# I2PC/xmipp3

Measured on AMD Instinct MI355X. Metric: particles/s projection-matched+reconstructed, 256x256 box, higher is better.
Workload: dtype f32 (coarse search, gridding) + f64 (exact re-score, shifts, finaliser)

## Files before the change

### xmipp3_amd/csrc/xh_pm.hip

```cpp
#include "xh_common.h"
#include "xh_fft.h"
#include "xh_fftreg.h"
#include "xh_plan.h"
#include "xh_bspline.h"
#include <algorithm>
#include <cmath>
#include <cstring>
#include <type_traits>

namespace {
const double kPI = 3.14159265358979323846;
const double kTWOPI = 6.2831853071795864769;

struct Layout {
    int D, Ri, Ro, nrings, nsamples, ncoef, N, nk;
    std::vector<int> nsam, soff, coff;
};

void make_layout(Layout &L, int D, int Ri, int Ro)
{
    L.D = D; L.Ri = Ri; L.Ro = Ro; L.nrings = Ro - Ri + 1;
    L.nsam.resize(L.nrings); L.soff.resize(L.nrings); L.coff.resize(L.nrings);
    L.nsamples = L.ncoef = 0;
    for (int r = 0; r < L.nrings; ++r) {
// ... 34 lines not shown
    int p0, np;
    int qoff, nq;
    int row0;
    int rowstride;
};
}

struct xh_pm {
    xh_ctx *ctx;
    Layout L;
    int nrefs, logM, M;
    double tau_rel, scale;
    size_t chunk_rows;
    XhBuf d_sin, d_cos, d_ringOfSample, d_nsam, d_soff, d_coff, d_rstart, d_ringW;
    XhBuf d_tw32, d_tw64;
    XhBuf d_refs64, d_refsB, d_refSigma, d_refCoef, d_refCoef32;
    XhBuf d_W32;
    XhBuf d_Wfull, d_vperm;
    int R1, R2, R3;
    XhBuf d_chirp, d_vhat;
    XhBuf d_csN;
    XhBuf d_WD64;
    XhBuf d_refScale;
    XhPlanBufs<double> planD;
    XhBuf d_coef32, d_polar32, d_A32, d_stat32;
    XhBuf d_trAngles;
    XhBuf d_trScale;
    XhBuf d_cellStart, d_cellSamples, d_cellOrg, d_cellData;
    int ncells;
    XhBuf d_coef64, d_polar64, d_A64, d_stat64;
    XhBuf d_raw, d_rowres, d_desc, d_nbr, d_poff;
    XhBuf d_ambList, d_ambSlot, d_candRow, d_candRes, d_counters, d_offs5d, d_thrLists;
    int ref_threads = 1;
    XhBuf d_t1, d_t2, d_t3;
    int64_t stat_rows, stat_resc_p, stat_resc_r;
    int coefFirst, coefCount;
    hipEvent_t ev[6] = {};
    double stage_ms[8];
    int store_cut;
    int s6_capture;
    int s6_captured;
    int s6_capturedN;
    int s6_fp32;
    double s6_eps;
    long long s6_flagged;
    XhBuf d_firTmp64;
    int tr_chunk_mb;
    int use_prune;
    int use_mask_lists;
    XhBuf d_bpart, d_rowBound, d_rowTail, d_topRows, d_thr, d_survList, d_survSpan, d_highStore;
    int group_high;
    int high_cap;
    int s6_layout;
    int low_pass;
    int64_t stat_pruned;
    int64_t stat_low_in, stat_low_out, stat_low_rows;
    int lastPruneRows;
    int lastLowPass;
    int adaptive_finish;
    int finish_dense;
    int stat_dense_chunks;
    int K0, K0auto, quadsLow;
    XhBuf d_bT, d_aT, d_kboundsLow, d_bTband;
    XhBuf d_firTmp, d_polarPart, d_trPart, d_listMask, d_s6Flag, d_s6List, d_s6Parts, d_s6Meta, d_s6Out;
    XhBuf d_qoff, d_Bpack, d_Apack, d_kbounds;
    int totalQuads;
    ~xh_pm()
    {
        (void)hipSetDevice(ctx->device);
        (void)hipStreamSynchronize(ctx->stream);
        for (hipEvent_t e : ev)
            if (e) (void)hipEventDestroy(e);
    }
};

__device__ __forceinline__ double d_block_sum(double v, double *red)
{
    for (int o = 32; o > 0; o >>= 1) v += __shfl_down(v, o, 64);
    const int lane = threadIdx.x & 63, wv = threadIdx.x >> 6;
    __syncthreads();
    if (lane == 0) red[wv] = v;
    __syncthreads();
    double t = 0;
    const int nw = (blockDim.x + 63) >> 6;
    for (int i = 0; i < nw; ++i) t += red[i];
    return t;
}

template <typename T>
__global__ void __launch_bounds__(256)
k_pm_polar(const T *__restrict__ coefs, T *__restrict__ polar, double *__restrict__ stat,
           const float *__restrict__ sinr, const float *__restrict__ cosr, const short *__restrict__ ringOf,
           const double *__restrict__ ringW, int D, int Ri, int nsamples, double xoff, double yoff,
           const int *__restrict__ count, int nt, const double *__restrict__ offs, int nparts, double *__restrict__ partial)
{
    __shared__ double red[8];
    const int slot = blockIdx.x / nparts, part = blockIdx.x - slot * nparts;
    if (count && slot / nt >= *count) return;
    const T *c = coefs + (size_t)(slot / nt) * D * D;
    if (offs) { xoff = offs[2 * (slot % nt)]; yoff = offs[2 * (slot % nt) + 1]; }
    const T minp = (T)(-(D / 2)), maxp = (T)(-(D / 2) + D - 1);
    const T eps = (T)1e-6;
    double sw = 0, swv = 0, swv2 = 0;
    const int per = (nsamples + nparts - 1) / nparts;
    const int iEnd = min(nsamples, (part + 1) * per);
    for (int i = part * per + threadIdx.x; i < iEnd; i += blockDim.x) {
        T xp = (T)sinr[i] + (T)xoff;
        T yp = (T)cosr[i] + (T)yoff;
        if (xp < minp - eps || xp > maxp + eps) xp = d_realwrap<T>(xp, minp - (T)0.5, maxp + (T)0.5);
        if (yp < minp - eps || yp > maxp + eps) yp = d_realwrap<T>(yp, minp - (T)0.5, maxp + (T)0.5);
        const T v = d_interp<T>(c, D, xp, yp);
        polar[(size_t)slot * nsamples + i] = v;
        const double w = ringW[ringOf[i]];
        const double dv = (double)v;
        sw += w; swv += w * dv; swv2 += w * dv * dv;
// ... 494 lines not shown
        for (int p = 0; p < PT; ++p)
#pragma unroll
            for (int q = 0; q < QT; ++q) {
                acc[p][q][0] = fmaf(a[p].x, b[q].x, acc[p][q][0]);
                acc[p][q][1] = fmaf(a[p].x, b[q].y, acc[p][q][1]);
                acc[p][q][2] = fmaf(a[p].y, b[q].x, acc[p][q][2]);
                acc[p][q][3] = fmaf(a[p].y, b[q].y, acc[p][q][3]);
            }
    }
#pragma unroll
    for (int p = 0; p < PT; ++p)
#pragma unroll
        for (int q = 0; q < QT; ++q)
            if (p < d.np && q < d.nq) {
                const size_t row = (size_t)d.row0 + (size_t)p * d.rowstride + q;
                raw[row * nk + k] = make_float4(acc[p][q][0], acc[p][q][1], acc[p][q][2], acc[p][q][3]);
            }
}


typedef float xh_f32x16 __attribute__((ext_vector_type(16)));

__global__ void k_pm_pack_tiles(const xh_cf *__restrict__ src, float4 *__restrict__ dst, const int *__restrict__ qoff,
                                const int *__restrict__ rstart, const int *__restrict__ coff, const int *__restrict__ nsam,
                                int nrings, int ncoef, int nk, int totalQuads, int nitems, const int *__restrict__ ids,
                                int quadLimit)
{
    const size_t gid = (size_t)blockIdx.x * blockDim.x + threadIdx.x;
    const int l = gid & 63;
    const size_t rest = gid >> 6;
    const int quad = rest % totalQuads;
    const int tile = rest / totalQuads;
    if ((size_t)tile * 16 >= (size_t)((nitems + 15) / 16) * 16) return;
    if (quad >= quadLimit) return;
    int lo = 0, hi = nk - 1;
    while (lo < hi) { const int mid = (lo + hi + 1) >> 1; if (qoff[mid] <= quad) lo = mid; else hi = mid - 1; }
    const int k = lo, q = quad - qoff[k];
    const int item = tile * 16 + ((l & 31) >> 1), part = l & 1;
    float v[4];
#pragma unroll
    for (int t = 0; t < 4; ++t) {
        const int ring = rstart[k] + 8 * q + 2 * t + (l >> 5);
        float x = 0.f;
        if (item < nitems && ring < nrings && k <= nsam[ring] / 2) {
            const int it = ids ? ids[item] : item;
            const xh_cf c = src[(size_t)it * ncoef + coff[ring] + k];
            x = part ? c.y : c.x;
        }
        v[t] = x;
    }
    dst[gid] = make_float4(v[0], v[1], v[2], v[3]);
}

#define XH_PW2 1
#define XH_KSPLIT 8
#define XH_CT_NQ 4
template <int PT, int QT, bool LDS = false>
__global__ void __launch_bounds__(64 * PT * QT)
k_pm_contract_mfma(const float4 *__restrict__ Apack, const float4 *__restrict__ Bpack, float4 *__restrict__ raw,
                   const int *__restrict__ qoff, const int *__restrict__ kbounds, int nk, int totalQuads, int nparticles,
                   int nq, int nqtiles, int nptiles, float2 *__restrict__ bpart, int rawStride, int kStore)
{
    static_assert(!LDS || (PT == 1 && XH_PW2 == 1 && XH_CT_NQ % QT == 0), "the LDS form shares one particle tile per workgroup");
    const int lane = threadIdx.x & 63, wv = threadIdx.x >> 6;
    int qtile = blockIdx.x * QT + wv % QT;
    const int ptile0 = (blockIdx.y * PT + wv / QT) * XH_PW2;
    const int kBeg = kbounds[blockIdx.z], kEnd = kbounds[blockIdx.z + 1];
    if (!LDS && qtile >= nqtiles) return;
    const int qtileStore = qtile;
    qtile = min(qtile, nqtiles - 1);
    const float4 *A[XH_PW2];
#pragma unroll
    for (int t = 0; t < XH_PW2; ++t) A[t] = Apack + (size_t)min(ptile0 + t, nptiles - 1) * totalQuads * 64 + lane;
    const float4 *B = Bpack + (size_t)qtile * totalQuads * 64 + lane;
    constexpr int STAGE_F4 = LDS ? (XH_CT_NQ + QT * XH_CT_NQ) * 64 : 1;
    __shared__ float4 sOp[2 * STAGE_F4];
    const unsigned sBase = LDS ? (unsigned)(uintptr_t)(const __attribute__((address_space(3))) float4 *)sOp : 0u;
    const int hi = lane >> 5, j = lane & 31;
    const int qj = j >> 1, odd = j & 1;
    const int q = qtileStore * 16 + qj;
    const int lastQuad = qoff[nk] - 1;
    float bndS[XH_PW2][4][2], bndM[XH_PW2][4][2];
#pragma unroll
    for (int t = 0; t < XH_PW2; ++t)
#pragma unroll
        for (int g = 0; g < 4; ++g) { bndS[t][g][0] = bndS[t][g][1] = 0.f; bndM[t][g][0] = bndM[t][g][1] = 0.f; }
    auto modulus = [&](const float4 &o, int k, float &bs, float &bm) {
        const float fsr = o.x - o.w, fsi = o.y + o.z, fmr = o.x + o.w, fmi = o.y - o.z;
        if (k == 0 || k == nk - 1) { bs += fabsf(fsr); bm += fabsf(fmr); }
        else { bs += 2.f * sqrtf(fsr * fsr + fsi * fsi); bm += 2.f * sqrtf(fmr * fmr + fmi * fmi); }
    };
    float4 a0[XH_PW2], a1[XH_PW2], b0, b1;
    const int qFirst = min(qoff[kBeg], lastQuad);
    int curStage = -1;
    const int wvq = __builtin_amdgcn_readfirstlane(wv % QT), qtileU = __builtin_amdgcn_readfirstlane(qtile);
    const int ptileU = __builtin_amdgcn_readfirstlane(min(ptile0, nptiles - 1));
    auto issueStage = [&](int st) {
        const unsigned buf = sBase + (unsigned)(st & 1) * (unsigned)(STAGE_F4 * 16);
        const unsigned off = (unsigned)lane * 16u;
#pragma unroll
        for (int jq = 0; jq < XH_CT_NQ; ++jq) {
            const int qd = min(qFirst + st * XH_CT_NQ + jq, lastQuad);
            const char *gb = reinterpret_cast<const char *>(Bpack) + ((size_t)qtileU * totalQuads + qd) * 1024;
            asm volatile("s_mov_b32 m0, %2\n\ts_nop 0\n\tglobal_load_lds_dwordx4 %0, %1" :: "v"(off), "s"(gb),
                         "s"(buf + (unsigned)(XH_CT_NQ + wvq * XH_CT_NQ + jq) * 1024u) : "memory");
            if (jq % QT == wvq) {
                const char *ga = reinterpret_cast<const char *>(Apack) + ((size_t)ptileU * totalQuads + qd) * 1024;
                asm volatile("s_mov_b32 m0, %2\n\ts_nop 0\n\tglobal_load_lds_dwordx4 %0, %1" :: "v"(off), "s"(ga), "s"(buf + (unsigned)jq * 1024u) : "memory");
            }
        }
    };
    auto fetch = [&](int qd, float4 (&av)[XH_PW2], float4 &bv) {
        if constexpr (!LDS) {
            bv = B[(size_t)qd * 64];
#pragma unroll
            for (int t = 0; t < XH_PW2; ++t) av[t] = A[t][(size_t)qd * 64];
        } else {
            const int rel = qd - qFirst, st = rel / XH_CT_NQ, jq = rel - st * XH_CT_NQ;
            if (st > curStage) {
                asm volatile("s_waitcnt vmcnt(0)" ::: "memory");
                __syncthreads();
                curStage = st;
                issueStage(st + 1);
            }
            const float4 *bufp = sOp + (size_t)(st & 1) * STAGE_F4;
            av[0] = bufp[jq * 64 + lane];
            bv = bufp[(XH_CT_NQ + wvq * XH_CT_NQ + jq) * 64 + lane];
        }
    };
    if constexpr (LDS) issueStage(0);
    fetch(qFirst, a0, b0);
    b1 = b0;
#pragma unroll
    for (int t = 0; t < XH_PW2; ++t) a1[t] = a0[t];
    for (int k0 = kBeg; k0 < kEnd; k0 += 4) {
        xh_f32x16 acc[XH_PW2][4];
#pragma unroll
        for (int kk = 0; kk < 4; ++kk) {
#pragma unroll
            for (int t = 0; t < XH_PW2; ++t)
#pragma unroll
                for (int e = 0; e < 16; ++e) acc[t][kk][e] = 0.f;
            const int k = k0 + kk;
            if (k < kEnd) {
                const int qb = qoff[k], qe = qoff[k + 1];
#define XH_CT_STEP(AC, BC, AN, BN, QN)                                                                        \
                {                                                                                              \
                    const int qn_ = (QN) <= lastQuad ? (QN) : lastQuad;                                        \
                    fetch(qn_, AN, BN);                                                                        \
                    __builtin_amdgcn_sched_barrier(0);                                                         \
                    _Pragma("unroll") for (int t = 0; t < XH_PW2; ++t) {                                       \
                        acc[t][kk] = __builtin_amdgcn_mfma_f32_32x32x2f32(AC[t].x, BC.x, acc[t][kk], 0, 0, 0); \
                        acc[t][kk] = __builtin_amdgcn_mfma_f32_32x32x2f32(AC[t].y, BC.y, acc[t][kk], 0, 0, 0); \
                        acc[t][kk] = __builtin_amdgcn_mfma_f32_32x32x2f32(AC[t].z, BC.z, acc[t][kk], 0, 0, 0); \
                        acc[t][kk] = __builtin_amdgcn_mfma_f32_32x32x2f32(AC[t].w, BC.w, acc[t][kk], 0, 0, 0); \
                    }                                                                                          \
                    __builtin_amdgcn_sched_barrier(0);                                                         \
                }
                for (int qd = qb; qd < qe; qd += 2) {
                    XH_CT_STEP(a0, b0, a1, b1, qd + 1)
                    if (qd + 1 < qe) XH_CT_STEP(a1, b1, a0, b0, qd + 2)
                }
#undef XH_CT_STEP
                if ((qe - qb) & 1) {
                    b0 = b1;
#pragma unroll
                    for (int t = 0; t < XH_PW2; ++t) a0[t] = a1[t];
                }
            }
        }
#pragma unroll
        for (int t = 0; t < XH_PW2; ++t)
#pragma unroll
        for (int g = 0; g < 4; ++g)
#pragma unroll
            for (int h2 = 0; h2 < 2; ++h2) {
                const int r0 = 4 * g + 2 * h2;
                const int pi = 4 * g + 2 * hi + h2;
                const int p = (ptile0 + t) * 16 + pi;
                float mine[4][2], theirs[2][2];
#pragma unroll
                for (int kk = 0; kk < 4; ++kk) { mine[kk][0] = acc[t][kk][r0]; mine[kk][1] = acc[t][kk][r0 + 1]; }
#pragma unroll
                for (int c = 0; c < 2; ++c) {
                    const float s0 = odd ? mine[0][c] : mine[2][c];
                    const float s1 = odd ? mine[1][c] : mine[3][c];
                    theirs[0][c] = __shfl_xor(s0, 1, 64);
                    theirs[1][c] = __shfl_xor(s1, 1, 64);
                }
                if (ptile0 + t < nptiles && p < nparticles && q < nq) {
                    float4 *dst = raw + ((size_t)p * nq + q) * rawStride;
                    const int kA = k0 + (odd ? 2 : 0);
                    float4 o0, o1;
                    if (!odd) {
                        o0 = make_float4(mine[0][0], theirs[0][0], mine[0][1], theirs[0][1]);
                        o1 = make_float4(mine[1][0], theirs[1][0], mine[1][1], theirs[1][1]);
                    } else {
                        o0 = make_float4(theirs[0][0], mine[2][0], theirs[0][1], mine[2][1]);
                        o1 = make_float4(theirs[1][0], mine[3][0], theirs[1][1], mine[3][1]);
                    }
                    if (kA < kEnd && kA < kStore) dst[kA] = o0;
                    if (kA + 1 < kEnd && kA + 1 < kStore) dst[kA + 1] = o1;
                    if (bpart) {
                        if (kA < kEnd) modulus(o0, kA, bndS[t][g][h2], bndM[t][g][h2]);
                        if (kA + 1 < kEnd) modulus(o1, kA + 1, bndS[t][g][h2], bndM[t][g][h2]);
                    }
                }
            }
    }
    if (bpart) {
        const size_t nrowsTotal = (size_t)nparticles * nq;
#pragma unroll
        for (int t = 0; t < XH_PW2; ++t)
#pragma unroll
            for (int g = 0; g < 4; ++g)
#pragma unroll
                for (int h2 = 0; h2 < 2; ++h2) {
                    const float bs = bndS[t][g][h2] + __shfl_xor(bndS[t][g][h2], 1, 64);
                    const float bm = bndM[t][g][h2] + __shfl_xor(bndM[t][g][h2], 1, 64);
                    const int p = (ptile0 + t) * 16 + 4 * g + 2 * hi + h2;
                    if (!odd && ptile0 + t < nptiles && p < nparticles && q < nq)
                        bpart[(size_t)blockIdx.z * nrowsTotal + (size_t)p * nq + q] = make_float2(bs, bm);
                }
    }
}

struct RowRes { float best; int idx; float second; int pad; };

__device__ __forceinline__ void d_top2_insert(float v, int i, float &b, int &bi, float &s)
{
    if (v > b || (v == b && i < bi)) { s = b; b = v; bi = i; }
    else if (v > s) s = v;
}

template <int LOGM>
__global__ void __launch_bounds__(256)
k_pm_idft_max(const float4 *__restrict__ raw, RowRes *__restrict__ res, const xh_cf *__restrict__ W,
              const xh_cf *__restrict__ chirp, const xh_cf *__restrict__ vhat, int N, int nk, int nrows, int lpb)
{
    extern __shared__ __align__(16) unsigned char smem[];
    xh_cf *s = reinterpret_cast<xh_cf *>(smem);
    constexpr int M = 1 << LOGM;
    const int tid = threadIdx.x, nth = blockDim.x;
    const int row0 = blockIdx.x * lpb;
    const int nl = min(lpb, nrows - row0);
    for (int i = tid; i < lpb * M; i += nth) s[i] = xh_cf{0.f, 0.f};
    __syncthreads();
    const int half = N / 2;
    for (int i = tid; i < nl * nk; i += nth) {
        const int l = i / nk, k = i - l * nk;
        const float4 q = raw[(size_t)(row0 + l) * nk + k];
        const float fsr = q.x - q.w, fsi = q.y + q.z;
        const float fmr = q.x + q.w, fmi = q.y - q.z;
        xh_cf *u = s + l * M;
        if (k == 0 || k == half) {
            u[k] = xh_cmul(xh_cf{fsr, fmr}, chirp[k]);
        } else {
            u[k] = xh_cmul(xh_cf{fsr - fmi, fsi + fmr}, chirp[k]);
            u[N - k] = xh_cmul(xh_cf{fsr + fmi, fmr - fsi}, chirp[N - k]);
        }
    }
    __syncthreads();
    xh_fft_dif<float, false>(s, LOGM, lpb, W, LOGM, tid, nth);
    for (int i = tid; i < lpb * M; i += nth) s[i] = xh_cmul(s[i], vhat[i & (M - 1)]);
    __syncthreads();
    xh_fft_dit<float, true>(s, LOGM, lpb, W, LOGM, tid, nth);
    __shared__ float rb[4 * 64], rs[4 * 64];
    __shared__ int ri[4 * 64];
    const int lane = tid & 63, wv = tid >> 6, nw = nth >> 6;
    for (int l = 0; l < nl; ++l) {
        float b = -3.0e38f, sec = -3.0e38f;
        int bi = 0x7fffffff;
        for (int i = tid; i < N; i += nth) {
            const xh_cf z = xh_cmul(s[l * M + i], chirp[i]);
            d_top2_insert(z.x, i, b, bi, sec);
            d_top2_insert(z.y, N + i, b, bi, sec);
// ... 2385 lines not shown
        XH_LAUNCH_CHECK();
        return XH_OK;
    }
    const size_t smem2 = sizeof(T) * ((L.N + 3) & ~3) + sizeof(xh_c2<T>) * L.N;
    hipLaunchKernelGGL((k_pm_ringdft<T>), dim3(L.nrings, (unsigned)nps), dim3(256), smem2, ctx->stream, (const T *)polarBuf.p,
                       (const double *)statBuf.p, (xh_c2<T> *)outBuf.p, (const xh_c2<T> *)twBuf.p,
                       (const int *)pm->d_nsam.p, (const int *)pm->d_soff.p, (const int *)pm->d_coff.p, L.nsamples,
                       L.ncoef, conjugate ? 1 : 0, d_count, nt);
    XH_LAUNCH_CHECK();
    return XH_OK;
}

template <typename T> static int upload(xh_ctx *ctx, XhBuf &b, const std::vector<T> &v)
{
    return xh_buf_upload(ctx, b, v.data(), sizeof(T) * v.size());
}

template <int LOGM>
static void launch_idft(xh_pm *pm, int nrows, int lpb, size_t smem)
{
    hipLaunchKernelGGL((k_pm_idft_max<LOGM>), dim3((nrows + lpb - 1) / lpb), dim3(256), smem, pm->ctx->stream,
                       (const float4 *)pm->d_raw.p, (RowRes *)pm->d_rowres.p, (const xh_cf *)pm->d_W32.p,
                       (const xh_cf *)pm->d_chirp.p, (const xh_cf *)pm->d_vhat.p, pm->L.N, pm->L.nk, nrows, lpb);
}
template <int LOGM>
static void launch_idft_dump(xh_pm *pm, float *d_out, size_t smem)
{
    hipLaunchKernelGGL((k_pm_idft_dump<LOGM>), dim3(1), dim3(256), smem, pm->ctx->stream, (const float4 *)pm->d_raw.p, d_out,
                       (const xh_cf *)pm->d_W32.p, (const xh_cf *)pm->d_chirp.p, (const xh_cf *)pm->d_vhat.p, pm->L.N,
                       pm->L.nk);
}

extern "C" {

static int set_k0(xh_pm *pm, int K0)
{
    const Layout &L = pm->L;
    K0 = std::max(4, std::min(L.nk, (K0 + 3) / 4 * 4));
    std::vector<int> qoff(L.nk + 1);
    XH_HIP(hipMemcpy(qoff.data(), pm->d_qoff.p, sizeof(int) * (L.nk + 1), hipMemcpyDeviceToHost));
    const int quads = qoff[K0];
    std::vector<int> kb(XH_KSPLIT + 1, K0);
    kb[0] = 0;
    for (int sidx = 1; sidx < XH_KSPLIT; ++sidx) {
        const int target = (int)((long long)quads * sidx / XH_KSPLIT);
        int k = 0;
        while (k < K0 && qoff[k] < target) ++k;
        kb[sidx] = std::min(K0, (k + 3) / 4 * 4);
    }
    XH_TRY(xh_buf_reserve(pm->ctx, pm->d_kboundsLow, sizeof(int) * kb.size()));
    XH_HIP(hipMemcpy(pm->d_kboundsLow.p, kb.data(), sizeof(int) * kb.size(), hipMemcpyHostToDevice));
    pm->K0 = K0;
    pm->quadsLow = quads;
    return XH_OK;
}

int xh_pm_create(xh_ctx *ctx, int32_t D, int32_t Ri, int32_t Ro, int32_t nrefs, const float *d_refs,
                 const double *h_Mctf, int32_t paddim, xh_pm **out)
{
    XH_CHECK(ctx && d_refs && out && nrefs > 0, XH_ERR_ARG, "xh_pm_create: bad argument");
    XH_CHECK(h_Mctf == nullptr || (paddim >= D && paddim <= 2048), XH_ERR_UNSUPPORTED,
             "xh_pm_create: the CTF filter size (paddim=%d) must lie in [image size %d, 2048]", paddim, D);
    if (Ri < 1) Ri = 1;
    if (Ro < 0) Ro = (D / 2) - 1;
    XH_CHECK(D >= 8 && Ro >= Ri && Ro < D, XH_ERR_ARG, "xh_pm_create: bad geometry D=%d Ri=%d Ro=%d", D, Ri, Ro);
    XH_HIP(hipSetDevice(ctx->device));
    std::unique_ptr<xh_pm> pm(new xh_pm);
    pm->ctx = ctx;
    pm->nrefs = nrefs;
    make_layout(pm->L, D, Ri, Ro);
    Layout &L = pm->L;
    XH_CHECK(L.nk <= 1024 && L.nrings <= 512, XH_ERR_UNSUPPORTED, "xh_pm_create: Ro=%d gives %d angular frequencies / %d rings; limits are 1024 / 512",
             Ro, L.nk, L.nrings);
    pm->M = 1;
    while (pm->M < 2 * L.N - 1) pm->M <<= 1;
    pm->logM = xh_ilog2(pm->M);
    XH_CHECK(pm->logM >= 6 && pm->logM <= 12, XH_ERR_UNSUPPORTED, "xh_pm_create: convolution length %d outside the supported 64..4096", pm->M);
    pm->scale = 0;
    for (int r = 0; r < L.nrings; ++r) pm->scale += 2. * kPI * (r + Ri);
    pm->tau_rel = D >= 128 ? 2e-6 : 3e-6;
    pm->s6_capture = 0;
    pm->s6_captured = 0;
    pm->s6_capturedN = 0;
    pm->s6_fp32 = 1;
    pm->s6_eps = 6.4e-6;
    pm->s6_flagged = 0;
    pm->use_prune = 1;
    pm->use_mask_lists = 1;
    pm->tr_chunk_mb = 0;
    pm->stat_pruned = 0;
    pm->lastPruneRows = 0;
    pm->adaptive_finish = 1;
    pm->group_high = 1;
    pm->low_pass = 1;
    pm->s6_layout = 1;
    pm->stat_low_in = pm->stat_low_out = pm->stat_low_rows = 0;
    pm->lastLowPass = 0;
    pm->high_cap = 0;
    pm->finish_dense = 0;
    pm->stat_dense_chunks = 0;
    pm->store_cut = 0;
    pm->chunk_rows = 0;
    pm->stat_rows = pm->stat_resc_p = pm->stat_resc_r = 0;
    pm->coefFirst = pm->coefCount = 0;
    for (int i = 0; i < 8; ++i) pm->stage_ms[i] = 0;
    for (int i = 0; i < 6; ++i) (void)hipEventCreate(&pm->ev[i]);
    {
        std::vector<float> sn(L.nsamples), cs(L.nsamples);
        std::vector<short> ringOf(L.nsamples), ringOfCoef(L.ncoef);
        std::vector<xh_cf> tw32(L.nsamples);
        std::vector<xh_cd> tw64(L.nsamples);
        for (int r = 0; r < L.nrings; ++r) {
            const float radius = r + Ri;
            const int n = L.nsam[r];
            const float dphi = kTWOPI / (float)n;
            for (int i = 0; i < n; ++i) {
                const float phi = i * dphi;
                sn[L.soff[r] + i] = std::sin(phi) * radius;
                cs[L.soff[r] + i] = std::cos(phi) * radius;
                ringOf[L.soff[r] + i] = (short)r;
                const long double a = -2.0L * 3.14159265358979323846264338327950288L * i / n;
                tw64[L.soff[r] + i] = xh_cd{(double)cosl(a), (double)sinl(a)};
                tw32[L.soff[r] + i] = xh_cf{(float)cosl(a), (float)sinl(a)};
            }
            for (int k = 0; k <= n / 2; ++k) ringOfCoef[L.coff[r] + k] = (short)r;
        }
        std::vector<int> rstart(L.nk);
        for (int k = 0; k < L.nk; ++k) {
            int r = 0;
            while (r < L.nrings && L.nsam[r] / 2 < k) ++r;
            rstart[k] = r;
        }
        const int M = pm->M, N = L.N;
        std::vector<xh_cf> W32(M / 2), chirp(N), vbr(M);
        for (int j = 0; j < M / 2; ++j) {
            const long double a = -2.0L * 3.14159265358979323846264338327950288L * j / M;
            W32[j] = xh_cf{(float)cosl(a), (float)sinl(a)};
        }
        std::vector<xh_cd> b(M, xh_cd{0., 0.});
        for (int n2 = 0; n2 < N; ++n2) {
            const long long q = ((long long)n2 * n2) % (2LL * N);
            const long double a = 3.14159265358979323846264338327950288L * (long double)q / (long double)N;
            chirp[n2] = xh_cf{(float)cosl(a), (float)sinl(a)};
            const xh_cd v{(double)cosl(a), (double)-sinl(a)};
            b[n2] = v;
            if (n2 > 0) b[M - n2] = v;
        }
        h_fft(b, false);
// ... 137 lines not shown
                                            pm->d_A64, pm->d_stat64, pm->d_tw64, true, 0., 0.));
                if (hipMemcpyAsync((xh_cd *)pm->d_refs64.p + (size_t)r0 * L.ncoef, pm->d_A64.p, sizeof(xh_cd) * (size_t)m * L.ncoef,
                                   hipMemcpyDeviceToDevice, ctx->stream) != hipSuccess ||
                    hipMemcpyAsync((double *)pm->d_refCoef.p + (size_t)r0 * D * D, pm->d_coef64.p, sizeof(double) * (size_t)m * D * D,
                                   hipMemcpyDeviceToDevice, ctx->stream) != hipSuccess ||
                    hipMemcpyAsync(stat.data(), pm->d_stat64.p, sizeof(double) * 2 * m, hipMemcpyDeviceToHost, ctx->stream) != hipSuccess ||
                    hipStreamSynchronize(ctx->stream) != hipSuccess) {
                    xh_set_error("xh_pm_create: reference library copy failed: %s", hipGetErrorString(hipGetLastError()));
                    return XH_ERR_HIP;
                }
                for (int i = 0; i < m; ++i) sig[r0 + i] = stat[2 * i + 1];
            }
            (void)hipStreamSynchronize(ctx->stream);
        }
        XH_CHECK(hipMemcpy(pm->d_refSigma.p, sig.data(), sizeof(double) * nrefs, hipMemcpyHostToDevice) == hipSuccess, XH_ERR_HIP,
                 "xh_pm_create: sigma upload failed");
        XH_TRY(xh_buf_alloc(ctx, pm->d_refScale, sizeof(int2) * nrefs));
        hipLaunchKernelGGL(k_pm_s6_norm_refs, dim3(nrefs), dim3(256), 0, ctx->stream, (const double *)pm->d_refCoef.p, D * D, (int2 *)pm->d_refScale.p);
        XH_CHECK(hipGetLastError() == hipSuccess, XH_ERR_HIP, "xh_pm_create: reference norms failed");
        {
            const size_t total = (size_t)nrefs * L.ncoef;
            hipLaunchKernelGGL(k_pm_pack_refs, dim3((unsigned)((total + 255) / 256)), dim3(256), 0, ctx->stream,
                               (const xh_cd *)pm->d_refs64.p, (xh_cf *)pm->d_refsB.p, (const short *)d_ringOfCoef.p, Ri, L.ncoef, total);
            XH_CHECK(hipGetLastError() == hipSuccess && hipStreamSynchronize(ctx->stream) == hipSuccess, XH_ERR_HIP, "xh_pm_create: pack kernel failed");
        }
        {
            std::vector<int> qoff(L.nk + 1);
            qoff[0] = 0;
            for (int k = 0; k < L.nk; ++k) qoff[k + 1] = qoff[k] + (L.nrings - rstart[k] + 7) / 8;
            pm->totalQuads = qoff[L.nk];
            XH_TRY(upload(ctx, pm->d_qoff, qoff));
            {
                std::vector<int> kb(XH_KSPLIT + 1, L.nk);
                kb[0] = 0;
                for (int sidx = 1; sidx < XH_KSPLIT; ++sidx) {
                    const int target = (int)((long long)pm->totalQuads * sidx / XH_KSPLIT);
                    int k = 0;
                    while (k < L.nk && qoff[k] < target) ++k;
                    kb[sidx] = std::min(L.nk, (k + 3) / 4 * 4);
                }
                XH_TRY(upload(ctx, pm->d_kbounds, kb));
            }
            const int ntiles = (nrefs + 15) / 16;
            const size_t nvec = (size_t)ntiles * pm->totalQuads * 64;
            XH_TRY(xh_buf_alloc(ctx, pm->d_Bpack, nvec * sizeof(float4)));
            {
                hipLaunchKernelGGL(k_pm_pack_tiles, dim3((unsigned)((nvec + 255) / 256)), dim3(256), 0, ctx->stream, (const xh_cf *)pm->d_refsB.p,
                                   (float4 *)pm->d_Bpack.p, (const int *)pm->d_qoff.p, (const int *)pm->d_rstart.p, (const int *)pm->d_coff.p,
                                   (const int *)pm->d_nsam.p, L.nrings, L.ncoef, L.nk, pm->totalQuads, nrefs, (const int *)nullptr, pm->totalQuads);
                XH_CHECK(hipGetLastError() == hipSuccess && hipStreamSynchronize(ctx->stream) == hipSuccess, XH_ERR_HIP, "xh_pm_create: operand packing failed");
            }
            pm->K0 = pm->K0auto = L.nk;
            pm->quadsLow = pm->totalQuads;
            XH_TRY(xh_buf_alloc(ctx, pm->d_bT, sizeof(float) * (size_t)L.nk * nrefs));
            {
                hipLaunchKernelGGL(k_pm_tail_norms, dim3((L.nk + 63) / 64, nrefs), dim3(64), 0, ctx->stream, (const xh_cf *)pm->d_refsB.p,
                                   (float *)pm->d_bT.p, (const int *)pm->d_coff.p, (const int *)pm->d_rstart.p, L.nrings, L.ncoef, L.nk, 0,
                                   nrefs, (size_t)1, (size_t)nrefs);
                std::vector<float> bT((size_t)L.nk * nrefs);
                XH_CHECK(hipGetLastError() == hipSuccess && hipMemcpy(bT.data(), pm->d_bT.p, pm->d_bT.bytes, hipMemcpyDeviceToHost) == hipSuccess, XH_ERR_HIP,
                         "xh_pm_create: reference norms failed");
                {
                    std::vector<double> mean(L.nk, 0.);
                    double all = 0;
                    for (int k = 0; k < L.nk; ++k) {
                        for (int r = 0; r < nrefs; ++r) mean[k] += bT[(size_t)k * nrefs + r];
                        all += mean[k];
                    }
                    double tailSum = 0;
                    int K0 = L.nk;
                    for (int k = L.nk - 1; k >= 0; --k) {
                        tailSum += mean[k];
                        if (!(tailSum <= 1e-5 * all)) break;
                        K0 = k;
                    }
                    K0 = std::min(L.nk, (K0 + 3) / 4 * 4);
                    if (K0 < 8) K0 = 8;
                    if (K0 > (int)(0.6 * L.nk)) K0 = L.nk;
                    pm->K0auto = K0;
                    XH_TRY(set_k0(pm.get(), K0));
                    const int nb = (L.nk + XH_TAIL_BAND - 1) / XH_TAIL_BAND;
                    std::vector<float> bb((size_t)nb * nrefs, 0.f);
                    for (int k = 0; k < L.nk; ++k)
                        for (int r = 0; r < nrefs; ++r) bb[(size_t)(k / XH_TAIL_BAND) * nrefs + r] += bT[(size_t)k * nrefs + r];
                    for (float &v : bb) v *= 1.000002f;
                    XH_TRY(upload(ctx, pm->d_bTband, bb));
                }
            }
        }
    }
    *out = pm.release();
    return XH_OK;
}

int xh_pm_destroy(xh_pm *pm)
{
    delete pm;
    return XH_OK;
}

int xh_pm_info(const xh_pm *pm, int32_t *N, int32_t *ncoef, int32_t *nsamples)
{
    XH_CHECK(pm, XH_ERR_ARG, "null handle");
    if (N) *N = pm->L.N;
    if (ncoef) *ncoef = pm->L.ncoef;
    if (nsamples) *nsamples = pm->L.nsamples;
    return XH_OK;
}

int xh_pm_set_option(xh_pm *pm, const char *name, double value)
{
    XH_CHECK(pm && name, XH_ERR_ARG, "null argument");
    if (!strcmp(name, "tau_rel")) pm->tau_rel = value;
    else if (!strcmp(name, "chunk_rows")) pm->chunk_rows = (size_t)value;
    else if (!strcmp(name, "s6_capture")) pm->s6_capture = (int)value;
    else if (!strcmp(name, "s6_fp32")) pm->s6_fp32 = (int)value;
    else if (!strcmp(name, "s6_eps")) pm->s6_eps = value;
    else if (!strcmp(name, "prune")) pm->use_prune = (int)value;
    else if (!strcmp(name, "mask_lists")) pm->use_mask_lists = (int)value;
    else if (!strcmp(name, "group_high")) pm->group_high = (int)value;
    else if (!strcmp(name, "low_pass")) pm->low_pass = (int)value;
    else if (!strcmp(name, "s6_layout")) pm->s6_layout = (int)value != 0;
    else if (!strcmp(name, "high_cap")) pm->high_cap = (int)value;
    else if (!strcmp(name, "adaptive_finish")) { pm->adaptive_finish = (int)value; pm->finish_dense = value >= 2; }
    else if (!strcmp(name, "threads")) {
        XH_CHECK(value >= 1 && value <= XH_MAX_ORIENT, XH_ERR_ARG, "xh_pm_set_option: threads in [1, %d]", XH_MAX_ORIENT);
        pm->ref_threads = (int)value;
    }
    else if (!strcmp(name, "tr_chunk_mb")) pm->tr_chunk_mb = (int)value;
    else if (!strcmp(name, "k0")) {
        XH_HIP(hipSetDevice(pm->ctx->device));
        XH_HIP(hipStreamSynchronize(pm->ctx->stream));
        XH_TRY(set_k0(pm, value <= 0 ? pm->K0auto : (int)value));
    }
    else { xh_set_error("xh_pm_set_option: unknown option %s", name); return XH_ERR_ARG; }
    return XH_OK;
}

int xh_pm_stage_ms(xh_pm *pm, double *h_ms, int32_t reset)
{
    XH_CHECK(pm && h_ms, XH_ERR_ARG, "null argument");
    for (int i = 0; i < 8; ++i) { h_ms[i] = pm->stage_ms[i]; if (reset) pm->stage_ms[i] = 0; }
    return XH_OK;
}

int xh_pm_two_level_cut(const xh_pm *pm, int32_t *K0, int32_t *nk)
{
    XH_CHECK(pm, XH_ERR_ARG, "null handle");
    if (K0) *K0 = pm->K0;
    if (nk) *nk = pm->L.nk;
    return XH_OK;
}

int xh_pm_rows_pruned(const xh_pm *pm, int64_t *rows_pruned)
{
    XH_CHECK(pm && rows_pruned, XH_ERR_ARG, "null argument");
    *rows_pruned = pm->stat_pruned;
    return XH_OK;
}

int xh_pm_last_coefficients(const xh_pm *pm, const float **d_coefs, int32_t *first, int32_t *count)
{
    XH_CHECK(pm && d_coefs && first && count, XH_ERR_ARG, "null argument");
    *d_coefs = pm->coefCount > 0 ? (const float *)pm->d_coef32.p : nullptr;
    *first = pm->coefFirst;
    *count = pm->coefCount;
    return XH_OK;
}

int xh_pm_last_stats(const xh_pm *pm, int64_t *rows, int64_t *rp, int64_t *rr)
{
    XH_CHECK(pm, XH_ERR_ARG, "null handle");
    if (rows) *rows = pm->stat_rows;
    if (rp) *rp = pm->stat_resc_p;
    if (rr) *rr = pm->stat_resc_r;
    return XH_OK;
}

static int run_rows(xh_pm *pm, int m, const std::vector<int> &poff, const int *d_ids, bool dense, int nq, hipEvent_t evMid = nullptr,
                    const RowMap *prune = nullptr, int nparticles = 0, float tau2 = 0.f, int *d_pruned = nullptr,
                    const unsigned *d_mask = nullptr, int maskW = 0, int listedRows = 0)
{
    xh_ctx *ctx = pm->ctx;
    const Layout &L = pm->L;
    const int nrows = poff[m];
    if (nrows == 0) return XH_OK;
    XH_TRY(xh_buf_reserve(ctx, pm->d_rowres, sizeof(RowRes) * (size_t)nrows));
    XH_CHECK(!dense || nq == pm->nrefs, XH_ERR_STATE, "xh_pm_match: internal error, a dense search covers the whole bank");
    std::vector<BlockDesc> desc;
    if (!dense) {
        for (int p = 0; p < m; ++p)
            for (int q0 = poff[p]; q0 < poff[p + 1]; q0 += 8) {
                BlockDesc d;
                d.p0 = p; d.np = 1; d.qoff = q0; d.nq = std::min(8, poff[p + 1] - q0);
                d.row0 = q0; d.rowstride = 0;
                desc.push_back(d);
            }
        XH_TRY(xh_buf_reserve(ctx, pm->d_desc, sizeof(BlockDesc) * desc.size()));
        XH_HIP(hipMemcpyAsync(pm->d_desc.p, desc.data(), sizeof(BlockDesc) * desc.size(), hipMemcpyHostToDevice, ctx->stream));
        XH_HIP(hipStreamSynchronize(ctx->stream));
    }
    const int nt = ((L.nk + 63) / 64) * 64;
    const bool pruning = dense && prune && pm->use_prune && pm->R1 && nparticles > 0 && nrows % nparticles == 0;
    XH_CHECK(!d_mask || pruning, XH_ERR_STATE, "xh_pm_match: internal error, a masked search must take the pruning path");
    if (pruning) XH_TRY(xh_buf_reserve(ctx, pm->d_bpart, sizeof(float2) * (size_t)XH_KSPLIT * nrows));
    const int K0 = pruning ? pm->K0 : L.nk;
    const bool boundsOnly = pruning && K0 >= L.nk && pm->store_cut >= 0 && pm->store_cut < L.nk;
    const int rawStride = boundsOnly ? pm->store_cut : std::min(K0, L.nk);
    XH_TRY(xh_buf_reserve(ctx, pm->d_raw, sizeof(float4) * std::max<size_t>(1, (size_t)nrows * rawStride)));
    XhHigh H;
    H.A = (const xh_cf *)pm->d_A32.p; H.B = (const xh_cf *)pm->d_refsB.p; H.coff = (const int *)pm->d_coff.p;
    H.rstart = (const int *)pm->d_rstart.p; H.nrings = L.nrings; H.ncoef = L.ncoef; H.K0 = boundsOnly ? rawStride : K0; H.nq = nq; H.zeroHigh = 0; H.rawStride = rawStride;
    H.nk = L.nk;
    H.highStore = nullptr; H.highCap = 0;
    if (dense) {
        const int ptiles = (m + 15) / 16, qtiles = (nq + 15) / 16;
        const size_t nvec = (size_t)ptiles * pm->totalQuads * 64;
        XH_TRY(xh_buf_reserve(ctx, pm->d_Apack, nvec * sizeof(float4)));
        hipLaunchKernelGGL(k_pm_pack_tiles, dim3((unsigned)((nvec + 255) / 256)), dim3(256), 0, ctx->stream, (const xh_cf *)pm->d_A32.p,
                           (float4 *)pm->d_Apack.p, (const int *)pm->d_qoff.p, (const int *)pm->d_rstart.p, (const int *)pm->d_coff.p,
                           (const int *)pm->d_nsam.p, L.nrings, L.ncoef, L.nk, pm->totalQuads, m, (const int *)nullptr,
                           K0 < L.nk ? pm->quadsLow : pm->totalQuads);
        XH_LAUNCH_CHECK();
        const int *kb = (const int *)(K0 < L.nk ? pm->d_kboundsLow.p : pm->d_kbounds.p);
        float2 *bpart = pruning ? (float2 *)pm->d_bpart.p : (float2 *)nullptr;
        if (K0 < L.nk)
            hipLaunchKernelGGL((k_pm_contract_mfma<1, 4, true>), dim3((qtiles + 3) / 4, ptiles, XH_KSPLIT), dim3(256), 0, ctx->stream,
                               (const float4 *)pm->d_Apack.p, (const float4 *)pm->d_Bpack.p, (float4 *)pm->d_raw.p, (const int *)pm->d_qoff.p,
                               kb, L.nk, pm->totalQuads, m, nq, qtiles, ptiles, bpart, rawStride, rawStride);
        else
            hipLaunchKernelGGL((k_pm_contract_mfma<1, 4>), dim3((qtiles + 3) / 4, (ptiles + XH_PW2 - 1) / XH_PW2, XH_KSPLIT), dim3(256), 0, ctx->stream,
                               (const float4 *)pm->d_Apack.p, (const float4 *)pm->d_Bpack.p, (float4 *)pm->d_raw.p, (const int *)pm->d_qoff.p,
                               kb, L.nk, pm->totalQuads, m, nq, qtiles, ptiles, bpart, rawStride, rawStride);
    } else
        hipLaunchKernelGGL((k_pm_contract<1, 8>), dim3((unsigned)desc.size()), dim3(nt), 0, ctx->stream,
                           (const BlockDesc *)pm->d_desc.p, (const xh_cf *)pm->d_A32.p, (const xh_cf *)pm->d_refsB.p, d_ids,
                           (float4 *)pm->d_raw.p, (const int *)pm->d_coff.p, (const int *)pm->d_rstart.p, L.nrings, L.ncoef, L.nk);
    XH_LAUNCH_CHECK();
    if (evMid) XH_HIP(hipEventRecord(evMid, ctx->stream));
    const int lpb = std::max(1, std::min(4, (60 * 1024) / (int)(pm->M * sizeof(xh_cf))));
    const size_t smem = (size_t)lpb * pm->M * sizeof(xh_cf);
    if (pm->R1) {
#define XH_IDFT3(A_, B_, C_)                                                                                  \
    hipLaunchKernelGGL((k_pm_idft_max3<A_, B_, C_>), dim3(grid), dim3(256), 0, ctx->stream, (const float4 *)pm->d_raw.p, \
                       (RowRes *)pm->d_rowres.p, (const xh_cf *)pm->d_Wfull.p, (const xh_cf *)pm->d_chirp.p,       \
                       (const xh_cf *)pm->d_vperm.p, L.N, L.nk, nr, rowList, H, nrDev)
#define XH_IDFT3_ANY()                                  \
    do {                                                \
        if (pm->logM == 9) XH_IDFT3(8, 8, 8);           \
        else if (pm->logM == 10) XH_IDFT3(16, 8, 8);    \
        else XH_IDFT3(16, 16, 8);                       \
    } while (0)
        int nr = nrows;
        const int *rowList = nullptr, *nrDev = nullptr;
        int grid;
        if (pruning) {
            XH_TRY(xh_buf_reserve(ctx, pm->d_rowBound, sizeof(float) * (size_t)nrows));
            XH_TRY(xh_buf_reserve(ctx, pm->d_rowTail, sizeof(float) * (size_t)nrows));
            XH_TRY(xh_buf_reserve(ctx, pm->d_topRows, sizeof(int) * (size_t)nparticles * XH_PRUNE_T));
            XH_TRY(xh_buf_reserve(ctx, pm->d_thr, sizeof(float) * (size_t)nparticles));
            XH_TRY(xh_buf_reserve(ctx, pm->d_aT, sizeof(float) * (size_t)m * L.nk));
            if (K0 < L.nk) {
                hipLaunchKernelGGL(k_pm_tail_norms, dim3((L.nk - K0 + 63) / 64, m), dim3(64), 0, ctx->stream, (const xh_cf *)pm->d_A32.p,
                                   (float *)pm->d_aT.p, (const int *)pm->d_coff.p, (const int *)pm->d_rstart.p, L.nrings, L.ncoef, L.nk, K0,
                                   m, (size_t)L.nk, (size_t)1);
                XH_LAUNCH_CHECK();
            }
            hipLaunchKernelGGL(k_pm_prune_plan, dim3(nparticles), dim3(256), 0, ctx->stream, (const float2 *)pm->d_bpart.p, XH_KSPLIT,
                               (size_t)nrows, *prune, (const double *)pm->d_refSigma.p, (const double *)pm->d_stat32.p,
                               (float *)pm->d_rowBound.p, (int *)pm->d_topRows.p, (const float *)pm->d_aT.p, (const float *)pm->d_bT.p,
                               K0, L.nk, pm->nrefs, (float *)pm->d_rowTail.p, d_mask, maskW, (const float *)pm->d_bTband.p, XH_TAIL_BAND);
            XH_LAUNCH_CHECK();
            nr = nparticles * XH_PRUNE_T;
            rowList = (const int *)pm->d_topRows.p;
            grid = std::max(8, std::min((nr + 3) / 4, ctx->num_cus * 8) / 8 * 8);
            H.zeroHigh = boundsOnly ? 0 : 1;
            XH_IDFT3_ANY();
            H.zeroHigh = 0;
            XH_LAUNCH_CHECK();
// ... 489 lines not shown
                           d_particles + (size_t)p0 * per, (const double *)pm->d_refCoef.p, d_refno + p0, d_psi + p0,
                           d_flip + p0, z, D, L.N);
        hipLaunchKernelGGL(k_pm_s6_scale, dim3(m), dim3(256), 0, ctx->stream, d_particles + (size_t)p0 * per, d_refno + p0, d_flip + p0,
                           (const int2 *)pm->d_refScale.p, (int)per, (int4 *)sc);
        hipLaunchKernelGGL(k_pm_s6_balance, dim3((unsigned)((per + 255) / 256), m), dim3(256), 0, ctx->stream, (const xh_cd *)z, w, sc, (int)per);
        XH_LAUNCH_CHECK();
        const size_t nlines = (size_t)m * D;
        hipLaunchKernelGGL((xh_k_fft_lines<double, false>), dim3((unsigned)((nlines + lpb - 1) / lpb)), dim3(256), smem, ctx->stream,
                           w, planD, nlines, (size_t)1, (size_t)D, (size_t)0, (size_t)1, lpb);
        XH_LAUNCH_CHECK();
        hipLaunchKernelGGL((xh_k_fft_lines<double, false>), dim3((unsigned)((nlines + lpb - 1) / lpb)), dim3(256), smem, ctx->stream,
                           w, planD, nlines, (size_t)D, per, (size_t)1, (size_t)D, lpb);
        XH_LAUNCH_CHECK();
        XH_TRY(xh_buf_reserve(ctx, pm->d_t3, sizeof(xh_cd) * per * chunk));
        xh_cd *pw = (xh_cd *)pm->d_t3.p;
        hipLaunchKernelGGL(k_pm_crosspower, dim3((unsigned)((per + 255) / 256), m), dim3(256), 0, ctx->stream, (const xh_cd *)w, pw, D, sc);
        XH_LAUNCH_CHECK();
        hipLaunchKernelGGL((xh_k_fft_lines<double, true>), dim3((unsigned)((nlines + lpb - 1) / lpb)), dim3(256), smem, ctx->stream,
                           pw, planD, nlines, (size_t)1, (size_t)D, (size_t)0, (size_t)1, lpb);
        XH_LAUNCH_CHECK();
        hipLaunchKernelGGL((xh_k_fft_lines<double, true>), dim3((unsigned)((nlines + lpb - 1) / lpb)), dim3(256), smem, ctx->stream,
                           pw, planD, nlines, (size_t)D, per, (size_t)1, (size_t)D, lpb);
        XH_LAUNCH_CHECK();
        hipLaunchKernelGGL(k_pm_bestshift<double>, dim3(m), dim3(256), 0, ctx->stream, (const double *)pw, 2, (const xh_cd *)z, d_refno + p0,
                           d_flip + p0, D, max_shift, d_sx + p0, d_sy + p0, d_cc + p0, (const XhTrPart *)nullptr, 0, sc);
        XH_LAUNCH_CHECK();
    }
    return XH_OK;
}

int xh_pm_debug_s6_maps(xh_pm *pm, int32_t n, double *h_maps)
{
    XH_CHECK(pm && h_maps && n > 0, XH_ERR_ARG, "xh_pm_debug_s6_maps: bad argument");
    XH_CHECK(pm->s6_captured && n <= pm->s6_capturedN, XH_ERR_STATE, "xh_pm_debug_s6_maps: no captured maps (set_option s6_capture, then xh_pm_translate)");
    XH_HIP(hipSetDevice(pm->ctx->device));
    const size_t tot = (size_t)n * pm->L.D * pm->L.D;
    XH_HIP(hipStreamSynchronize(pm->ctx->stream));
    if (pm->s6_captured == 64) { XH_HIP(hipMemcpy(h_maps, pm->d_t3.p, tot * sizeof(double), hipMemcpyDeviceToHost)); return XH_OK; }
    std::vector<float> tmp(tot);
    XH_HIP(hipMemcpy(tmp.data(), pm->d_t3.p, tot * sizeof(float), hipMemcpyDeviceToHost));
    for (size_t i = 0; i < tot; ++i) h_maps[i] = tmp[i];
    return XH_OK;
}

int xh_pm_get_option(const xh_pm *pm, const char *name, double *value)
{
    XH_CHECK(pm && name && value, XH_ERR_ARG, "xh_pm_get_option: null argument");
    if (!strcmp(name, "tau_rel")) *value = pm->tau_rel;
    else if (!strcmp(name, "s6_eps")) *value = pm->s6_eps;
    else if (!strcmp(name, "adaptive_finish")) *value = pm->adaptive_finish;
    else if (!strcmp(name, "dense_chunks")) *value = pm->stat_dense_chunks;
    else if (!strcmp(name, "low_pass")) *value = pm->low_pass;
    else if (!strcmp(name, "s6_layout")) *value = pm->s6_layout;
    else if (!strcmp(name, "low_pass_rows_in")) *value = (double)pm->stat_low_in;
    else if (!strcmp(name, "low_pass_rows_out")) *value = (double)pm->stat_low_out;
    else if (!strcmp(name, "low_pass_rows_transformed")) *value = (double)pm->stat_low_rows;
    else { xh_set_error("xh_pm_get_option: unknown option %s", name); return XH_ERR_ARG; }
    return XH_OK;
}

int xh_pm_debug_prepare(xh_pm *pm, const float *d_particles, int32_t n, int32_t precision, double *h_coefs, double *h_sigma)
{
    XH_CHECK(pm && d_particles && h_coefs && h_sigma && n > 0, XH_ERR_ARG, "bad argument");
    XH_HIP(hipSetDevice(pm->ctx->device));
    xh_ctx *ctx = pm->ctx;
    const Layout &L = pm->L;
    std::vector<double> stat(2 * (size_t)n);
    if (precision == 64) {
        XH_TRY(run_prep<double>(pm, d_particles, true, nullptr, n, nullptr, pm->d_coef64, pm->d_polar64, pm->d_A64, pm->d_stat64,
                                pm->d_tw64, false, 0., 0.));
        XH_HIP(hipMemcpyAsync(h_coefs, pm->d_A64.p, sizeof(xh_cd) * (size_t)n * L.ncoef, hipMemcpyDeviceToHost, ctx->stream));
        XH_HIP(hipMemcpyAsync(stat.data(), pm->d_stat64.p, sizeof(double) * 2 * n, hipMemcpyDeviceToHost, ctx->stream));
        XH_HIP(hipStreamSynchronize(ctx->stream));
    } else {
        XH_TRY(run_prep<float>(pm, d_particles, true, nullptr, n, nullptr, pm->d_coef32, pm->d_polar32, pm->d_A32, pm->d_stat32,
                               pm->d_tw32, false, 0., 0.));
        std::vector<float> tmp(2 * (size_t)n * L.ncoef);
        XH_HIP(hipMemcpyAsync(tmp.data(), pm->d_A32.p, sizeof(xh_cf) * (size_t)n * L.ncoef, hipMemcpyDeviceToHost, ctx->stream));
        XH_HIP(hipMemcpyAsync(stat.data(), pm->d_stat32.p, sizeof(double) * 2 * n, hipMemcpyDeviceToHost, ctx->stream));
        XH_HIP(hipStreamSynchronize(ctx->stream));
        for (size_t i = 0; i < tmp.size(); ++i) h_coefs[i] = tmp[i];
    }
    for (int i = 0; i < n; ++i) h_sigma[i] = stat[2 * i + 1];
    return XH_OK;
}

int xh_pm_debug_ref(xh_pm *pm, int32_t ref, double *h_coefs, double *h_sigma)
{
    XH_CHECK(pm && h_coefs && h_sigma && ref >= 0 && ref < pm->nrefs, XH_ERR_ARG, "bad argument");
    XH_HIP(hipSetDevice(pm->ctx->device));
    xh_ctx *ctx = pm->ctx;
    XH_HIP(hipMemcpyAsync(h_coefs, (const xh_cd *)pm->d_refs64.p + (size_t)ref * pm->L.ncoef, sizeof(xh_cd) * pm->L.ncoef,
                          hipMemcpyDeviceToHost, ctx->stream));
    XH_HIP(hipMemcpyAsync(h_sigma, (const double *)pm->d_refSigma.p + ref, sizeof(double), hipMemcpyDeviceToHost, ctx->stream));
    XH_HIP(hipStreamSynchronize(ctx->stream));
    return XH_OK;
}

int xh_pm_debug_corr_rows(xh_pm *pm, const float *d_particle, int32_t ref, int32_t precision, double *h_corr2N)
{
    XH_CHECK(pm && d_particle && h_corr2N && ref >= 0 && ref < pm->nrefs, XH_ERR_ARG, "bad argument");
    XH_HIP(hipSetDevice(pm->ctx->device));
    xh_ctx *ctx = pm->ctx;
    const Layout &L = pm->L;
    const int N = L.N;
    int h_ids[1] = {ref};
// ... 60 lines not shown
```

Baseline: 128,200.

## Walk all k-slices in one MFMA workgroup and pack low-band tiles through LDS

Adds an s2_form path, on by default, for the low-frequency contraction. Each workgroup of the LDS MFMA kernel now walks all eight k-slices in sequence instead of launching one grid layer per slice, so the stage pipeline stays primed and per-slice launch and prologue work is avoided. A waves-per-eu hint is added for this path. It also adds a dedicated pack kernel that stages particle coefficients through shared memory to write the packed A tiles with coalesced stores; the cost is a grid with z-dimension one, which may reduce parallelism for small particle counts.

After: 128,800, median of 6. No clear change (+0.5%).

```diff
diff --git a/xmipp3_amd/csrc/xh_pm.hip b/xmipp3_amd/csrc/xh_pm.hip
--- a/xmipp3_amd/csrc/xh_pm.hip
+++ b/xmipp3_amd/csrc/xh_pm.hip
@@ -110,6 +110,7 @@
     int group_high;
     int high_cap;
     int s6_layout;
+    int s2_form;
     int low_pass;
     int64_t stat_pruned;
     int64_t stat_low_in, stat_low_out, stat_low_rows;
@@ -118,7 +119,7 @@
     int adaptive_finish;
     int finish_dense;
     int stat_dense_chunks;
-    int K0, K0auto, quadsLow;
+    int K0, K0auto, quadsLow, quadsLowMax;
     XhBuf d_bT, d_aT, d_kboundsLow, d_bTband;
     XhBuf d_firTmp, d_polarPart, d_trPart, d_listMask, d_s6Flag, d_s6List, d_s6Parts, d_s6Meta, d_s6Out;
     XhBuf d_qoff, d_Bpack, d_Apack, d_kbounds;
@@ -719,20 +720,62 @@
     dst[gid] = make_float4(v[0], v[1], v[2], v[3]);
 }
 
+#define XH_PL_LD 260
+__global__ void __launch_bounds__(256)
+k_pm_pack_tiles_low(const xh_cf *__restrict__ src, float4 *__restrict__ dst, const int *__restrict__ qoff, const int *__restrict__ rstart,
+                    const int *__restrict__ coff, const int *__restrict__ nsam, int nrings, int ncoef, int totalQuads, int nitems, int K0)
+{
+    __shared__ __align__(16) float s[32 * XH_PL_LD];
+    const int q = blockIdx.x, tile = blockIdx.y, kc = blockIdx.z * 32;
+    const int tid = threadIdx.x;
+    {
+        const int kl = tid & 31, k = kc + kl;
+        const bool kin = k < K0 && qoff[k] + q < qoff[k + 1];
+        const int r0 = kin ? rstart[k] + 8 * q : 0;
+        const int rq = tid >> 5, ring = r0 + rq;
+        const bool rin = kin && ring < nrings && k <= nsam[min(ring, nrings - 1)] / 2;
+        const xh_cf *p = src + (rin ? coff[ring] + k : 0);
+        xh_cf c[16];
+#pragma unroll
+        for (int it = 0; it < 16; ++it) c[it] = p[(size_t)min(tile * 16 + it, nitems - 1) * ncoef];
+#pragma unroll
+        for (int it = 0; it < 16; ++it)
+            if (!rin || tile * 16 + it >= nitems) c[it] = xh_cf{0.f, 0.f};
+        float *d = s + kl * XH_PL_LD + 32 * (rq & 1) * 4 + (rq >> 1);
+#pragma unroll
+        for (int it = 0; it < 16; ++it) {
+            d[it * 8] = c[it].x;
+            d[it * 8 + 4] = c[it].y;
+        }
+    }
+    __syncthreads();
+    const int l = tid & 63;
+    for (int kk = tid >> 6; kk < 32; kk += 4) {
+        const int k = kc + kk;
+        if (k >= K0 || qoff[k] + q >= qoff[k + 1]) continue;
+        dst[((size_t)tile * totalQuads + qoff[k] + q) * 64 + l] = *reinterpret_cast<const float4 *>(s + kk * XH_PL_LD + l * 4);
+    }
+}
+
 #define XH_PW2 1
 #define XH_KSPLIT 8
 #define XH_CT_NQ 4
-template <int PT, int QT, bool LDS = false>
-__global__ void __launch_bounds__(64 * PT * QT)
+#ifndef XH_S2_WALK_WAVES
+#define XH_S2_WALK_WAVES 3
+#endif
+template <int PT, int QT, bool LDS = false, bool WALK = false>
+__global__ void __launch_bounds__(64 * PT * QT) __attribute__((amdgpu_waves_per_eu(WALK ? XH_S2_WALK_WAVES : 1)))
 k_pm_contract_mfma(const float4 *__restrict__ Apack, const float4 *__restrict__ Bpack, float4 *__restrict__ raw,
                    const int *__restrict__ qoff, const int *__restrict__ kbounds, int nk, int totalQuads, int nparticles,
                    int nq, int nqtiles, int nptiles, float2 *__restrict__ bpart, int rawStride, int kStore)
 {
     static_assert(!LDS || (PT == 1 && XH_PW2 == 1 && XH_CT_NQ % QT == 0), "the LDS form shares one particle tile per workgroup");
+    static_assert(!WALK || LDS, "walking the slices keeps the stage pipeline of the LDS form running");
     const int lane = threadIdx.x & 63, wv = threadIdx.x >> 6;
     int qtile = blockIdx.x * QT + wv % QT;
     const int ptile0 = (blockIdx.y * PT + wv / QT) * XH_PW2;
-    const int kBeg = kbounds[blockIdx.z], kEnd = kbounds[blockIdx.z + 1];
+    const int sliceFirst = WALK ? 0 : (int)blockIdx.z, sliceEnd = WALK ? XH_KSPLIT : (int)blockIdx.z + 1;
+    int kBeg = kbounds[sliceFirst], kEnd = kbounds[sliceFirst + 1];
     if (!LDS && qtile >= nqtiles) return;
     const int qtileStore = qtile;
     qtile = min(qtile, nqtiles - 1);
@@ -800,6 +843,9 @@
     b1 = b0;
 #pragma unroll
     for (int t = 0; t < XH_PW2; ++t) a1[t] = a0[t];
+#pragma unroll 1
+    for (int slice = sliceFirst; slice < sliceEnd; ++slice) {
+    if (slice > sliceFirst) { kBeg = kEnd; kEnd = kbounds[slice + 1]; }
     for (int k0 = kBeg; k0 < kEnd; k0 += 4) {
         xh_f32x16 acc[XH_PW2][4];
 #pragma unroll
@@ -887,8 +933,10 @@
                     const float bm = bndM[t][g][h2] + __shfl_xor(bndM[t][g][h2], 1, 64);
                     const int p = (ptile0 + t) * 16 + 4 * g + 2 * hi + h2;
                     if (!odd && ptile0 + t < nptiles && p < nparticles && q < nq)
-                        bpart[(size_t)blockIdx.z * nrowsTotal + (size_t)p * nq + q] = make_float2(bs, bm);
+                        bpart[(size_t)slice * nrowsTotal + (size_t)p * nq + q] = make_float2(bs, bm);
+                    bndS[t][g][h2] = bndM[t][g][h2] = 0.f;
                 }
+    }
     }
 }
 
@@ -3380,6 +3428,8 @@
     XH_HIP(hipMemcpy(pm->d_kboundsLow.p, kb.data(), sizeof(int) * kb.size(), hipMemcpyHostToDevice));
     pm->K0 = K0;
     pm->quadsLow = quads;
+    pm->quadsLowMax = 0;
+    for (int k = 0; k < K0; ++k) pm->quadsLowMax = std::max(pm->quadsLowMax, qoff[k + 1] - qoff[k]);
     return XH_OK;
 }
 
@@ -3422,6 +3472,7 @@
     pm->group_high = 1;
     pm->low_pass = 1;
     pm->s6_layout = 1;
+    pm->s2_form = 1;
     pm->stat_low_in = pm->stat_low_out = pm->stat_low_rows = 0;
     pm->lastLowPass = 0;
     pm->high_cap = 0;
@@ -3665,6 +3716,7 @@
             }
             pm->K0 = pm->K0auto = L.nk;
             pm->quadsLow = pm->totalQuads;
+            pm->quadsLowMax = 0;
             XH_TRY(xh_buf_alloc(ctx, pm->d_bT, sizeof(float) * (size_t)L.nk * nrefs));
             {
                 hipLaunchKernelGGL(k_pm_tail_norms, dim3((L.nk + 63) / 64, nrefs), dim3(64), 0, ctx->stream, (const xh_cf *)pm->d_refsB.p,
@@ -3734,6 +3786,7 @@
     else if (!strcmp(name, "group_high")) pm->group_high = (int)value;
     else if (!strcmp(name, "low_pass")) pm->low_pass = (int)value;
     else if (!strcmp(name, "s6_layout")) pm->s6_layout = (int)value != 0;
+    else if (!strcmp(name, "s2_form")) pm->s2_form = (int)value != 0;
     else if (!strcmp(name, "high_cap")) pm->high_cap = (int)value;
     else if (!strcmp(name, "adaptive_finish")) { pm->adaptive_finish = (int)value; pm->finish_dense = value >= 2; }
     else if (!strcmp(name, "threads")) {
@@ -3830,14 +3883,23 @@
         const int ptiles = (m + 15) / 16, qtiles = (nq + 15) / 16;
         const size_t nvec = (size_t)ptiles * pm->totalQuads * 64;
         XH_TRY(xh_buf_reserve(ctx, pm->d_Apack, nvec * sizeof(float4)));
-        hipLaunchKernelGGL(k_pm_pack_tiles, dim3((unsigned)((nvec + 255) / 256)), dim3(256), 0, ctx->stream, (const xh_cf *)pm->d_A32.p,
-                           (float4 *)pm->d_Apack.p, (const int *)pm->d_qoff.p, (const int *)pm->d_rstart.p, (const int *)pm->d_coff.p,
-                           (const int *)pm->d_nsam.p, L.nrings, L.ncoef, L.nk, pm->totalQuads, m, (const int *)nullptr,
-                           K0 < L.nk ? pm->quadsLow : pm->totalQuads);
+        if (K0 < L.nk && pm->s2_form && pm->quadsLowMax > 0)
+            hipLaunchKernelGGL(k_pm_pack_tiles_low, dim3(pm->quadsLowMax, ptiles, (K0 + 31) / 32), dim3(256), 0, ctx->stream,
+                               (const xh_cf *)pm->d_A32.p, (float4 *)pm->d_Apack.p, (const int *)pm->d_qoff.p, (const int *)pm->d_rstart.p,
+                               (const int *)pm->d_coff.p, (const int *)pm->d_nsam.p, L.nrings, L.ncoef, pm->totalQuads, m, K0);
+        else
+            hipLaunchKernelGGL(k_pm_pack_tiles, dim3((unsigned)((nvec + 255) / 256)), dim3(256), 0, ctx->stream, (const xh_cf *)pm->d_A32.p,
+                               (float4 *)pm->d_Apack.p, (const int *)pm->d_qoff.p, (const int *)pm->d_rstart.p, (const int *)pm->d_coff.p,
+                               (const int *)pm->d_nsam.p, L.nrings, L.ncoef, L.nk, pm->totalQuads, m, (const int *)nullptr,
+                               K0 < L.nk ? pm->quadsLow : pm->totalQuads);
         XH_LAUNCH_CHECK();
         const int *kb = (const int *)(K0 < L.nk ? pm->d_kboundsLow.p : pm->d_kbounds.p);
         float2 *bpart = pruning ? (float2 *)pm->d_bpart.p : (float2 *)nullptr;
-        if (K0 < L.nk)
+        if (K0 < L.nk && pm->s2_form)
+            hipLaunchKernelGGL((k_pm_contract_mfma<1, 4, true, true>), dim3((qtiles + 3) / 4, ptiles, 1), dim3(256), 0, ctx->stream,
+                               (const float4 *)pm->d_Apack.p, (const float4 *)pm->d_Bpack.p, (float4 *)pm->d_raw.p, (const int *)pm->d_qoff.p,
+                               kb, L.nk, pm->totalQuads, m, nq, qtiles, ptiles, bpart, rawStride, rawStride);
+        else if (K0 < L.nk)
             hipLaunchKernelGGL((k_pm_contract_mfma<1, 4, true>), dim3((qtiles + 3) / 4, ptiles, XH_KSPLIT), dim3(256), 0, ctx->stream,
                                (const float4 *)pm->d_Apack.p, (const float4 *)pm->d_Bpack.p, (float4 *)pm->d_raw.p, (const int *)pm->d_qoff.p,
                                kb, L.nk, pm->totalQuads, m, nq, qtiles, ptiles, bpart, rawStride, rawStride);
@@ -4433,6 +4495,7 @@
     else if (!strcmp(name, "dense_chunks")) *value = pm->stat_dense_chunks;
     else if (!strcmp(name, "low_pass")) *value = pm->low_pass;
     else if (!strcmp(name, "s6_layout")) *value = pm->s6_layout;
+    else if (!strcmp(name, "s2_form")) *value = pm->s2_form;
     else if (!strcmp(name, "low_pass_rows_in")) *value = (double)pm->stat_low_in;
     else if (!strcmp(name, "low_pass_rows_out")) *value = (double)pm->stat_low_out;
     else if (!strcmp(name, "low_pass_rows_transformed")) *value = (double)pm->stat_low_rows;
```
